# SuperScientificSoftwareLaboratory/TileSpMV

Measured on AMD Instinct MI355X. Metric: fp64 SpMV GFLOP/s (y = A*x, tiled format), higher is better.
Workload: dtype f64; 1 GPU; laplacian4096; rows=16777216, cols=16777216, nnz=83869696, partition=tile-row blocks, nnz-balanced, 1 rank(s), y_combine=none, tiles=5234176, x_panel_merge=0, x_slice_passes=0

## Files before the change

### tilespmv_amd/csrc/hip_plan.h

```cpp
#pragma once
#include <cstdint>

#include "host_util.h"

namespace tilespmv {

constexpr unsigned DESC_FMT_MASK = 7u;
constexpr unsigned DESC_FMT_NOP = 7u;
constexpr unsigned DESC_EOR = 8u;
constexpr int DESC_P1_SHIFT = 4;
constexpr int DESC_P2_SHIFT = 12;

#if defined(TILESPMV_F32)
struct ERec { unsigned v, w; };
#else
struct ERec { unsigned lo, hi, w; };
#endif
constexpr int ECHUNK = 64;
constexpr int SMALL_GRID_WORKGROUPS = 128;
constexpr int FB_DEST_BITS = 11;

struct Task {
    int tile_begin, tile_end;
    long long val_off;
    long long idx_off;
    int row;
    int partial;
};

struct FixRow { int row, first, count, pad; };

struct DevPlan {
    const uint2 *desc;
    const val_t *val;
    const unsigned char *idx;
    const Task *task;
    int ntasks;
    int rowA, colA;
    val_t *partial;
    const FixRow *fix;
    int nfix;
    const FixRow *fix_late;
    int nfix_late;
    const int4 *f_blk;
    const ERec *f_rec;
    const unsigned *f_base;
    int f_nblk;
    int f_ordered;
    int f_row0;
    int f_rows;
};

constexpr int FB_ROWS = 2048;
constexpr int FB_CAP = 6144;
constexpr int STRIP_MAX_ROWS = 8;
constexpr unsigned UNIT_EOR = 1u;
constexpr int UNIT_ROW_SHIFT = 1;
constexpr unsigned UNIT_ROWUNIT = 16u;
constexpr int UNIT_SHIFT_SHIFT = 29;
constexpr int ABSORB_SHIFT_MIN = -3, ABSORB_SHIFT_MAX = 3;
constexpr unsigned UNIT_DERIVED_CODE = 4u;
constexpr int UNIT_GROUP = 16 / (int)sizeof(val_t);
constexpr int UNIT_GROUP_NARROW = 4;
constexpr long long NT_STREAM_MIN_BYTES = 400ll << 20;
constexpr int DICT_MAX_BITS = 10;
constexpr int UNIT_FLAG_SHIFT = 24;

struct UDesc { unsigned w0, n0, n1; };

constexpr int POOL_KR_SHIFT = 28;
constexpr unsigned POOL_BASE_MASK = (1u << POOL_KR_SHIFT) - 1u;
constexpr int POOL_WORD_KR_SHIFT = 30;
__host__ __device__ inline int pool_word_base_bits(int npatterns)
{
    int ib = 1;
    while ((1 << ib) < npatterns) ib++;
    return POOL_WORD_KR_SHIFT - ib;
}
constexpr int POOL_MIN_FILL = sizeof(val_t) == 8 ? 12 : 10;
#ifndef TILESPMV_POOL_STRIP_ROWS
#define TILESPMV_POOL_STRIP_ROWS 4
#endif
constexpr int POOL_STRIP_ROWS = TILESPMV_POOL_STRIP_ROWS;
struct URow { unsigned r0, r1; };
constexpr unsigned POOL_WIDE_WINDOW = 256;
constexpr double POOL_WIDE_MAX_LINES = 3.5;

struct STask {
    int unit_begin, unit_end;
    int coo_begin, coo_end;
    int row;
    int partial;
    unsigned nounit_mask;
    int nrows;
};

struct DevStream {
    const UDesc *udesc;
    const URow *urow;
    const uint4 *ucol;
    const uint4 *pdict;
    int pooled;
    const val_t *uval;
    const val_t *cval;
    const int *ccol;
    const unsigned char *crow;
    const STask *task;
    int ntasks;
    int coo_heavy_min;
    int coo_ordered;
    int y_streaming;
    const int4 *wg_coo;
    const ERec *grec;
    const unsigned *gbase;
    int dest_bits;
    const uint4 *udict;
    int cb_bits;
    int nt_stream;
    int uval_narrow;
    const int *panel_off;
    int x_panels;
    int panel_merge;
    int n_groups;
    int slice_passes;
    int slice_ct;
    const UDesc *udesc_cb;
    const FixRow *ifix;
    unsigned *ifix_count;
};

struct DenseRow { int row, tile_begin, tile_end, partial; };
__host__ __device__ constexpr int dense_slot(int r, int c)
{
    return sizeof(val_t) == 8 ? ((c & 3) >> 1) * 128 + ((c >> 2) * 16 + r) * 2 + (c & 1) : ((c >> 2) * 16 + r) * 4 + (c & 3);
}

struct DevDense {
    const int *cb;
    const val_t *val;
    const DenseRow *rows;
    int nrows;
};

inline void tile_stream_sizes(int fmt, int p1, int p2, int *nv, int *ni)
{
    switch (fmt) {
    case TILESPMV_FMT_CSR: *nv = p1; *ni = 16 + (p1 + 1) / 2; break;
    case TILESPMV_FMT_COO: *nv = p1; *ni = p1; break;
    case TILESPMV_FMT_ELL: *nv = 16 * p1; *ni = 8 * p1; break;
    case TILESPMV_FMT_HYB: *nv = 16 * p1 + p2; *ni = 8 * p1 + p2; break;
    case TILESPMV_FMT_DNS: *nv = 256; *ni = 0; break;
    case TILESPMV_FMT_DNSROW: *nv = 16 * p1; *ni = p1; break;
    case TILESPMV_FMT_DNSCOL: *nv = 16 * p1; *ni = p1; break;
    default: *nv = 0; *ni = 0; break;
    }
}

hipError_t launch_units_half(const DevPlan &P, const DevStream &S, int entry_mode, int wg_strips, int lds_pad_bytes, int xcd_chunk, const val_t *x, val_t *y, hipStream_t st);

}
```

### tilespmv_amd/csrc/hip_units_kernel.h

```cpp
#pragma once
#include <hip/hip_runtime.h>

#include <type_traits>

#include "hip_plan.h"

namespace tilespmv {

typedef double lacc_t;

template <int CTRL>
__device__ __forceinline__ double dpp_mov(double v)
{
    int lo = __double2loint(v), hi = __double2hiint(v);
    lo = __builtin_amdgcn_update_dpp(0, lo, CTRL, 0xF, 0xF, false);
    hi = __builtin_amdgcn_update_dpp(0, hi, CTRL, 0xF, 0xF, false);
    return __hiloint2double(hi, lo);
}
template <int CTRL>
__device__ __forceinline__ float dpp_mov(float v)
{
    return __int_as_float(__builtin_amdgcn_update_dpp(0, __float_as_int(v), CTRL, 0xF, 0xF, false));
}
template <class T>
__device__ __forceinline__ T strip_allreduce(T v)
{
    v += dpp_mov<0x128>(v);
    v += dpp_mov<0x124>(v);
    v += dpp_mov<0x122>(v);
    v += dpp_mov<0x121>(v);
    return v;
}

__device__ __forceinline__ void wave_lds_fence()
{
    __builtin_amdgcn_fence(__ATOMIC_ACQ_REL, "wavefront");
    __builtin_amdgcn_wave_barrier();
}


template <bool NT, class T>
__device__ __forceinline__ T stream_load(const T *p)
{
    if constexpr (NT) return __builtin_nontemporal_load(p);
    else return *p;
}

__device__ __forceinline__ uint4 load_udesc(const UDesc *__restrict__ d, int i)
{
    const UDesc u = d[i];
    return make_uint4(u.w0, u.n0, u.w0, u.n1);
}

__device__ __forceinline__ uint4 load_udesc_raw(const UDesc *__restrict__ d, int i)
{
    const UDesc u = d[i];
    return make_uint4(u.w0, u.n0, u.n1, 0u);
}
__device__ __forceinline__ uint4 udesc_park_form(const uint4 raw) { return make_uint4(raw.x, raw.y, raw.x, raw.z); }

__device__ __forceinline__ uint4 udict_of(const DevStream &S, unsigned w) { return S.udict[(w << 5) >> (5 + S.cb_bits)]; }
__device__ __forceinline__ uint2 pool_desc(const DevStream &S, int i)
{
    const int b = S.cb_bits;
    if (b > 0) {
        const unsigned a = reinterpret_cast<const unsigned *>(S.udesc)[i];
        return make_uint2((a & ((1u << b) - 1u)) | ((a >> POOL_WORD_KR_SHIFT) << POOL_KR_SHIFT), (a << (32 - POOL_WORD_KR_SHIFT)) >> (32 - POOL_WORD_KR_SHIFT + b));
    }
    return reinterpret_cast<const uint2 *>(S.udesc)[i];
}
__device__ __forceinline__ uint4 udesc_expand(const DevStream &S, unsigned w, uint4 pat)
{
    const unsigned w0 = (w & ((1u << S.cb_bits) - 1u)) | ((w >> 27) << UNIT_FLAG_SHIFT) | pat.z;
    return make_uint4(w0, pat.x, w0, pat.y);
}
template <class X>
__device__ __forceinline__ X unit_x_use(X gathered, X prev, unsigned w0, int r)
{
    const X up = dpp_mov<0x12F>(prev);
    return ((w0 >> UNIT_SHIFT_SHIFT) == UNIT_DERIVED_CODE && r != 15) ? up : gathered;
}
__device__ __forceinline__ long long unit_x_base(unsigned w0) { return (long long)(w0 & 0xFFFFFFu) * 16 + ((int)w0 >> UNIT_SHIFT_SHIFT); }
__device__ __forceinline__ int unit_x_base32(unsigned w0) { return (int)((w0 & 0xFFFFFFu) << 4) + ((int)w0 >> UNIT_SHIFT_SHIFT); }
__device__ __forceinline__ unsigned x_index32(int base, unsigned off, int xlast) { return (unsigned)min(base + (int)off, xlast); }

constexpr int DCHUNK = 16;
typedef unsigned v4u_t __attribute__((ext_vector_type(4)));
typedef unsigned v2u_t __attribute__((ext_vector_type(2)));
#ifndef NT_Y
#define NT_Y 1
#endif
#ifndef WCOO_HEAVY_CT
#define WCOO_HEAVY_CT 6
#endif
#ifndef MV_MIN_WAVES
#define MV_MIN_WAVES 6
#endif
#ifndef ECOO2_MIN_WAVES
#define ECOO2_MIN_WAVES 6
#endif
#ifndef TILESPMV_UB
#define TILESPMV_UB 4
#endif
#ifndef UNITS_MIN_WAVES
#define UNITS_MIN_WAVES 8
#endif
#ifndef UNIT_X32
#define UNIT_X32 1
#endif
#ifndef UNIT_TAIL_HOT
#define UNIT_TAIL_HOT 1
#endif
#ifndef POOL_ECOO2_MIN_WAVES
#define POOL_ECOO2_MIN_WAVES 5
#endif
#ifndef POOL_MIN_WAVES
#define POOL_MIN_WAVES 7
#endif

__device__ __forceinline__ val_t erec_val(const ERec &r)
{
#if defined(TILESPMV_F32)
    return __uint_as_float(r.v);
#else
    return __hiloint2double((int)r.hi, (int)r.lo);
#endif
}

template <int CT>
__device__ __forceinline__ void wave_entry_trips(const DevStream &S, const val_t *__restrict__ x, lacc_t *swave, int lane, int gb, int ge, int chunk0, int cfirst)
{
    const int db = S.dest_bits;
    const unsigned dmask = (1u << db) - 1u;
    const int clast = chunk0 + ((ge - 1 - gb) >> 6);
    for (int e0 = gb + 64 * cfirst; e0 < ge; e0 += 64 * CT) {
        ERec rr[CT]; unsigned cb[CT]; val_t xx[CT];
#pragma unroll
        for (int q = 0; q < CT; q++) {
            rr[q] = S.grec[min(e0 + 64 * q + lane, ge - 1)];
            cb[q] = S.gbase[__builtin_amdgcn_readfirstlane(min(chunk0 + ((e0 - gb) >> 6) + q, clast))];
        }
#pragma unroll
        for (int q = 0; q < CT; q++) xx[q] = x[(size_t)(cb[q] + (rr[q].w >> db))];
#pragma unroll
        for (int q = 0; q < CT; q++)
            if (e0 + 64 * q + lane < ge) atomicAdd(&swave[rr[q].w & dmask], (lacc_t)(erec_val(rr[q]) * xx[q]));
    }
}

#ifndef WG_TRIP_PIPE
#define WG_TRIP_PIPE 0
#endif

template <int CT, int NT, bool NTL>
__device__ __forceinline__ void wg_entry_trips(const ERec *__restrict__ rec, const unsigned *__restrict__ base, int chunk0, int db, bool ordered,
                                               const val_t *__restrict__ x, lacc_t *sy, int tid, int gb, int ge, int gs = -1)
{
    if (gs < 0) gs = gb;
    const int e_first = gb + ((gs - gb) & ~63);
    const unsigned dmask = (1u << db) - 1u;
    const int wave = tid >> 6;
    const int clast = chunk0 + ((ge - 1 - gb) >> 6);
    ERec rr[CT]; unsigned cb[CT];
    auto load_trip = [&](int e0, ERec (&r)[CT], unsigned (&c)[CT]) {
#pragma unroll
        for (int q = 0; q < CT; q++) {
            if constexpr (NTL) {
                const unsigned *pw = reinterpret_cast<const unsigned *>(&rec[min(e0 + NT * q + tid, ge - 1)]);
                unsigned *rw = reinterpret_cast<unsigned *>(&r[q]);
#pragma unroll
                for (int z = 0; z < (int)(sizeof(ERec) / 4); z++) rw[z] = __builtin_nontemporal_load(pw + z);
            } else r[q] = rec[min(e0 + NT * q + tid, ge - 1)];
            c[q] = base[__builtin_amdgcn_readfirstlane(min(chunk0 + ((e0 - gb) >> 6) + (NT / 64) * q + wave, clast))];
        }
    };
    if (e_first < ge) load_trip(e_first, rr, cb);
    for (int e0 = e_first; e0 < ge; e0 += NT * CT) {
        val_t xx[CT];
        if (!WG_TRIP_PIPE && e0 > e_first) load_trip(e0, rr, cb);
#pragma unroll
        for (int q = 0; q < CT; q++) xx[q] = x[(size_t)(cb[q] + (rr[q].w >> db))];
        ERec rn[CT]; unsigned cn[CT];
        if (WG_TRIP_PIPE) load_trip(min(e0 + NT * CT, gb + (ge - 1 - gb) / (NT * CT) * (NT * CT)), rn, cn);
        if (ordered) {
            for (int w = 0; w < NT / 64; w++) {
                if (wave == w) {
#pragma unroll
                    for (int q = 0; q < CT; q++)
                        if (e0 + NT * q + tid < ge && e0 + NT * q + tid >= gs) atomicAdd(&sy[rr[q].w & dmask], (lacc_t)(erec_val(rr[q]) * xx[q]));
                }
                __syncthreads();
            }
        } else {
#pragma unroll
            for (int q = 0; q < CT; q++)
                if (e0 + NT * q + tid < ge && e0 + NT * q + tid >= gs) atomicAdd(&sy[rr[q].w & dmask], (lacc_t)(erec_val(rr[q]) * xx[q]));
        }
        if (WG_TRIP_PIPE) {
#pragma unroll
            for (int q = 0; q < CT; q++) { rr[q] = rn[q]; cb[q] = cn[q]; }
        }
    }
}

extern __shared__ __attribute__((aligned(16))) unsigned char s_dyn[];
#if defined(UNITS_KERNEL) != defined(UNITS_NARROW_FORM)
#error "hip_units_kernel.h: define UNITS_KERNEL and UNITS_NARROW_FORM together (or neither: k_units, floats)"
#endif
#ifndef UNITS_KERNEL
#define UNITS_KERNEL k_units
#define UNITS_NARROW_FORM 1
#endif
template <int UB, int ECOO, int GPB, bool CD, bool NTS, bool POOL = false, bool WIDE = false, bool NARROW = false>
__global__ __launch_bounds__(16 * GPB, ECOO == 1 ? 4 : ECOO == 2 ? (POOL ? POOL_ECOO2_MIN_WAVES : NARROW && UNITS_NARROW_FORM == 2 ? UNITS_MIN_WAVES : ECOO2_MIN_WAVES) : POOL ? (WIDE ? 6 : POOL_MIN_WAVES) : UNITS_MIN_WAVES) void UNITS_KERNEL(DevStream S, int rowA, int colA, int xcd_chunk, val_t *__restrict__ partial,
                                               const val_t *__restrict__ x, val_t *__restrict__ y)
{
    constexpr int VFORM = NARROW ? UNITS_NARROW_FORM : 0;
    static_assert(VFORM >= 0 && VFORM <= 2, "UNITS_NARROW_FORM: 1 or 2");
    static_assert(!NARROW || (sizeof(val_t) == 8 && !POOL && ECOO != 1 && GPB == 16 && NTS), "narrow values: fp64 classic plans, entry mode 0 / 2, 16 strips, nontemporal streams");
    constexpr int G = NARROW ? UNIT_GROUP_NARROW : UNIT_GROUP;
    static_assert(DCHUNK % UB == 0 && UB % G == 0, "a batch never straddles a descriptor chunk and is whole value groups");
    static_assert(GPB == 16 || (GPB == 32 && ECOO == 2) || (GPB == 8 && ECOO != 2 && !NTS), "512-thread workgroups exist for the workgroup entry mode only, 128-thread ones for small grids without it");
    static_assert(!(NTS && ECOO == 1), "nontemporal streams: large plans only (entry mode 1 = small grids)");
    static_assert(!POOL || GPB == 16 || GPB == 8, "pooled plans: 256-thread workgroups (128 on small grids)");
    static_assert(!WIDE || (POOL && !CD), "wide windows: pooled plans, 12-B descriptors + 16 B of column offsets");
    constexpr int GROUPS_PER_BLOCK = GPB;
    constexpr int SROWS = POOL ? POOL_STRIP_ROWS : STRIP_MAX_ROWS;
    constexpr bool NT = NTS;
#ifndef TILESPMV_NT_DESC
#define TILESPMV_NT_DESC 0
#endif
#ifndef TILESPMV_NT_COO0
#define TILESPMV_NT_COO0 0
#endif
    constexpr bool NT_DESC = NTS && TILESPMV_NT_DESC, NT_COO0 = NTS && TILESPMV_NT_COO0;
    constexpr bool PCOPY = POOL && sizeof(val_t) == 4;
    constexpr int SLAB = GROUPS_PER_BLOCK * SROWS * 16;
    __shared__ lacc_t s_yall[SLAB + (PCOPY ? SLAB + 16 : 0)];
    lacc_t (*s_y)[SROWS][16] = reinterpret_cast<lacc_t (*)[SROWS][16]>(&s_yall[0]);
    lacc_t *s_y1 = &s_yall[PCOPY ? SLAB + 16 : 0];
    __shared__ uint4 s_d[GROUPS_PER_BLOCK][DCHUNK];
    __shared__ uint2 s_r[POOL && !WIDE ? GROUPS_PER_BLOCK : 1][POOL && !WIDE ? DCHUNK : 1];
    __shared__ uint4 s_c[WIDE ? GROUPS_PER_BLOCK : 1][WIDE ? DCHUNK : 1];
    const int tid = threadIdx.x, r = tid & 15, g = tid >> 4;
    unsigned bid = blockIdx.x;
    if (xcd_chunk > 0) {
        const unsigned C = (unsigned)xcd_chunk, W = 8u * C, win = bid / W, off = bid % W, k = off & 7u;
        if ((win + 1) * W <= gridDim.x) bid = win * W + k * C + (off >> 3);
    }
    const long long task_id = (long long)bid * GROUPS_PER_BLOCK + g;
    const bool have = task_id < S.ntasks;
    constexpr bool WCOO = ECOO == 1;
    if (ECOO == 1) { if ((long long)bid * GROUPS_PER_BLOCK + (g & ~3) >= S.ntasks) return; }
    else if (ECOO == 0 && !have) return;
    int4 t0 = make_int4(0, 0, 0, 0), t1 = make_int4(0, -1, 0, 0);
    if (have) {
        t0 = reinterpret_cast<const int4 *>(S.task)[task_id * 2];
        t1 = reinterpret_cast<const int4 *>(S.task)[task_id * 2 + 1];
    }
    const int unit_begin = t0.x, unit_end = t0.y, coo_begin = t0.z, coo_end = t0.w;
    const int row0 = t1.x, part = t1.y, nrows = t1.w;
    const unsigned nounit = (unsigned)t1.z;
    const bool side = POOL || coo_end > coo_begin;
    if constexpr (POOL) {
        for (int k = 0; k < nrows; k++) { s_y[g][k][r] = 0; if constexpr (PCOPY) s_y1[(g * SROWS + k) * 16 + r] = 0; }
        wave_lds_fence();
    }
    typedef std::conditional_t<VFORM == 2, _Float16, std::conditional_t<VFORM == 1, float, val_t>> sval_t;
    typedef sval_t grp_t __attribute__((ext_vector_type(G)));
    const grp_t *__restrict__ ugrp = reinterpret_cast<const grp_t *>(S.uval) + r;
    const int last = unit_end - 1;
    const int last_grp = unit_begin + (unit_end - 1 - unit_begin) / G * G;
    const bool have_units = unit_begin < unit_end;
    const long long xlast = (long long)colA - 1;
    const int xlast32 = colA - 1;
    const int ncoo = coo_end - coo_begin;
    uint4 dcur = make_uint4(0u, 0u, 0u, 0u), dnext = dcur;
    uint2 rcur = make_uint2(0u, 0u), rnext = rcur;
    const uint2 *__restrict__ urw = reinterpret_cast<const uint2 *>(S.urow);
    uint4 ccur = make_uint4(0u, 0u, 0u, 0u), cnext = ccur;
    unsigned wnn = 0;
    const unsigned *__restrict__ udw = reinterpret_cast<const unsigned *>(S.udesc);
    uint2 wnn2 = make_uint2(0u, 0u);
    val_t v[UB];
    auto unit_prologue = [&]() {
        if (have_units) {
            if constexpr (CD && POOL) {
                const uint2 a = pool_desc(S, min(unit_begin + r, last)), b = pool_desc(S, min(unit_begin + DCHUNK + r, last));
                dcur.x = a.x; dcur.y = a.y; dnext.x = b.x; dnext.y = b.y;
            } else if constexpr (CD) {
                dcur.x = stream_load<NT_DESC>(udw + min(unit_begin + r, last));
                dnext.x = stream_load<NT_DESC>(udw + min(unit_begin + DCHUNK + r, last));
            } else {
                dcur = load_udesc_raw(S.udesc, min(unit_begin + r, last));
                dnext = load_udesc_raw(S.udesc, min(unit_begin + DCHUNK + r, last));
                if constexpr (WIDE) { ccur = S.ucol[min(unit_begin + r, last)]; cnext = S.ucol[min(unit_begin + DCHUNK + r, last)]; }
                else if constexpr (POOL) { rcur = urw[min(unit_begin + r, last)]; rnext = urw[min(unit_begin + DCHUNK + r, last)]; }
            }
#pragma unroll
            for (int k = 0; k < UB; k += G) {
                const grp_t pv = stream_load<NT>(ugrp + (long long)min(unit_begin + k, last_grp) * (16 / G));
#pragma unroll
                for (int q = 0; q < G; q++) v[k + q] = pv[q];
            }
        }
    };

    const uint2 *sd = reinterpret_cast<const uint2 *>(&s_d[g][0]) + (r >> 3);
    uint2 d[UB];
    unsigned rw[UB];
    val_t xv[UB];
    const unsigned *sr = reinterpret_cast<const unsigned *>(&s_r[POOL && !WIDE ? g : 0][0]) + (r >> 3);
    const unsigned char *sc = reinterpret_cast<const unsigned char *>(&s_c[WIDE ? g : 0][0]) + r;
    auto park_first = [&]() {
        if constexpr (CD && POOL) {
            const uint4 p0 = S.pdict[dcur.y], p1 = S.pdict[dnext.y];
            wnn2 = pool_desc(S, min(unit_begin + 2 * DCHUNK + r, last));
            s_d[g][r] = make_uint4(dcur.x, p0.x, dcur.x, p0.y); s_r[g][r] = make_uint2(p0.z, p0.w);
            dnext = make_uint4(dnext.x, p1.x, 0u, p1.y); rnext = make_uint2(p1.z, p1.w);
        } else if constexpr (CD) {
            const uint4 p0 = udict_of(S, dcur.x), p1 = udict_of(S, dnext.x);
            wnn = stream_load<NT_DESC>(udw + min(unit_begin + 2 * DCHUNK + r, last));
            dnext.y = p1.x; dnext.z = p1.z; dnext.w = p1.y;
            s_d[g][r] = udesc_expand(S, dcur.x, p0);
        } else s_d[g][r] = udesc_park_form(dcur);
        if constexpr (WIDE) s_c[g][r] = ccur;
        else if constexpr (POOL && !CD) s_r[g][r] = rcur;
    };
    auto fetch_batch = [&](int j0) {
#pragma unroll
        for (int k = 0; k < UB; k++) d[k] = sd[2 * (j0 + k)];
        if constexpr (WIDE) {
#pragma unroll
            for (int k = 0; k < UB; k++) rw[k] = d[k].y;
#pragma unroll
            for (int k = 0; k < UB; k++) {
                if constexpr (UNIT_X32) xv[k] = x[x_index32((int)(d[k].x & POOL_BASE_MASK), sc[16 * (j0 + k)], xlast32)];
                else xv[k] = x[min((long long)(d[k].x & POOL_BASE_MASK) + (long long)sc[16 * (j0 + k)], xlast)];
            }
            return;
        }
        if constexpr (POOL) {
#pragma unroll
            for (int k = 0; k < UB; k++) rw[k] = sr[2 * (j0 + k)];
#pragma unroll
            for (int k = 0; k < UB; k++) {
                if constexpr (UNIT_X32) xv[k] = x[x_index32((int)(d[k].x & POOL_BASE_MASK), (d[k].y >> (28 - 4 * (r & 7))) & 15u, xlast32)];
                else xv[k] = x[min((long long)(d[k].x & POOL_BASE_MASK) + (long long)((d[k].y >> (28 - 4 * (r & 7))) & 15u), xlast)];
            }
            return;
        }
#pragma unroll
        for (int k = 0; k < UB; k++) {
            const unsigned fl = d[k].x >> 24;
            const unsigned nib = (fl & UNIT_ROWUNIT) ? (unsigned)r : (d[k].y >> (28 - 4 * (r & 7))) & 15u;
            if ((d[k].x >> UNIT_SHIFT_SHIFT) == UNIT_DERIVED_CODE && r != 15) xv[k] = 0;
            else if constexpr (UNIT_X32) xv[k] = x[x_index32(unit_x_base32(d[k].x), nib, xlast32)];
            else xv[k] = x[min(unit_x_base(d[k].x) + nib, xlast)];
        }
    };

    if constexpr (ECOO == 2) {
        const int4 wr = S.wg_coo[bid];
        if (wr.y > wr.x) {
            if (side) for (int k = 0; k < nrows; k++) s_y[g][k][r] = 0;
            __syncthreads();
        } else if ((S.panel_merge > 0 || S.slice_passes > 0) && side) {
            for (int k = 0; k < nrows; k++) s_y[g][k][r] = 0;
            wave_lds_fence();
        }
        constexpr bool LATE_PROLOGUE = VFORM == 2;
        if constexpr (!LATE_PROLOGUE) unit_prologue();
        if (wr.y > wr.x) {
            int ge = wr.y;
            if (GPB == 16 && S.panel_merge > 0) ge = S.panel_off[(size_t)bid * (size_t)(S.x_panels + 1) + (size_t)min(S.x_panels, S.panel_merge)];
            if (GPB == 16 && S.slice_passes > 0) ge = wr.x;
            wg_entry_trips<WCOO_HEAVY_CT, 16 * GPB, NTS>(S.grec, S.gbase, wr.z, S.dest_bits, S.coo_ordered != 0, x, &s_y[0][0][0], tid, wr.x, ge);
            __syncthreads();
        }
        if constexpr (LATE_PROLOGUE) unit_prologue();
    } else if constexpr (WCOO) {
        constexpr int CT = 6;
        const int lane = tid & 63;
        const int4 wr = S.wg_coo[(long long)bid * (GROUPS_PER_BLOCK / 4) + (g >> 2)];
        const int tot = wr.y - wr.x;
        lacc_t *swave = &s_y[g & ~3][0][0];
        unit_prologue();
        ERec rr[CT]; unsigned cbase[CT]; val_t xx[CT];
        const int db = S.dest_bits;
        if (tot > 0) {
            if (side) for (int k = 0; k < nrows; k++) s_y[g][k][r] = 0;
            const int clast = wr.z + ((tot - 1) >> 6);
#pragma unroll
            for (int q = 0; q < CT; q++) {
                rr[q] = S.grec[min(wr.x + 64 * q + lane, wr.y - 1)];
                cbase[q] = S.gbase[__builtin_amdgcn_readfirstlane(min(wr.z + q, clast))];
            }
        }
        if (have_units) {
            park_first();
            wave_lds_fence();
            fetch_batch(0);
        } else if (tot > 0) wave_lds_fence();
        if (tot > 0) {
            const unsigned dmask = (1u << db) - 1u;
#pragma unroll
            for (int q = 0; q < CT; q++) xx[q] = x[(size_t)(cbase[q] + (rr[q].w >> db))];
#pragma unroll
            for (int q = 0; q < CT; q++)
                if (wr.x + 64 * q + lane < wr.y) atomicAdd(&swave[rr[q].w & dmask], (lacc_t)(erec_val(rr[q]) * xx[q]));
            if (tot > 64 * CT) wave_entry_trips<CT>(S, x, swave, lane, wr.x, wr.y, wr.z, CT);
            wave_lds_fence();
        }
    } else {
    constexpr int CT = 6;
    const bool coo_heavy = ncoo > S.coo_heavy_min;
    if (side) {
        for (int k = 0; k < nrows; k++) s_y[g][k][r] = 0;
        wave_lds_fence();
    }
    if (coo_heavy) {
        for (int e0 = coo_begin; e0 < coo_end; e0 += 16 * CT) {
            unsigned rb[CT]; int cc[CT]; val_t cv[CT], xx[CT];
#pragma unroll
            for (int q = 0; q < CT; q++) {
                const int e = min(e0 + 16 * q + r, coo_end - 1);
                rb[q] = S.crow[e]; cc[q] = S.ccol[e]; cv[q] = S.cval[e];
            }
#pragma unroll
            for (int q = 0; q < CT; q++) xx[q] = x[cc[q]];
#pragma unroll
            for (int q = 0; q < CT; q++)
                if (e0 + 16 * q + r < coo_end) atomicAdd(&s_y[g][rb[q] >> 4][rb[q] & 15u], (lacc_t)(cv[q] * xx[q]));
        }
        wave_lds_fence();
    }
    unsigned rb0 = 0; int cc0 = 0; val_t cv0 = 0;
    const bool coo0 = side && !coo_heavy && (coo_begin + r < coo_end);
    if (coo0) { rb0 = stream_load<NT_COO0>(S.crow + coo_begin + r); cc0 = stream_load<NT_COO0>(S.ccol + coo_begin + r); cv0 = stream_load<NT_COO0>(S.cval + coo_begin + r); }
    unit_prologue();
    if (side && !coo_heavy) {
        if (coo0) atomicAdd(&s_y[g][rb0 >> 4][rb0 & 15u], (lacc_t)(cv0 * x[cc0]));
        for (int e0 = coo_begin + 16; e0 < coo_end; e0 += 64) {
            unsigned rb[4]; int cc[4]; val_t cv[4], xx[4];
#pragma unroll
            for (int q = 0; q < 4; q++) {
                const int e = min(e0 + 16 * q + r, coo_end - 1);
                rb[q] = S.crow[e]; cc[q] = S.ccol[e]; cv[q] = S.cval[e];
            }
#pragma unroll
            for (int q = 0; q < 4; q++) xx[q] = x[cc[q]];
#pragma unroll
            for (int q = 0; q < 4; q++)
                if (e0 + 16 * q + r < coo_end) atomicAdd(&s_y[g][rb[q] >> 4][rb[q] & 15u], (lacc_t)(cv[q] * xx[q]));
        }
        wave_lds_fence();
    }
    }

    val_t acc = 0;
    auto retire = [&](val_t prod, unsigned flags, unsigned word1) {
        if constexpr (POOL) {
            const unsigned dest = ((flags >> (POOL_KR_SHIFT - 24)) & 7u) * 16u + ((word1 >> (28 - 4 * (r & 7))) & 15u);
            if constexpr (PCOPY) atomicAdd(((r & 1) ? s_y1 : &s_y[0][0][0]) + g * (SROWS * 16) + dest, (lacc_t)prod);
            else atomicAdd(&s_y[g][0][0] + dest, (lacc_t)prod);
            return;
        }
        if (flags & UNIT_ROWUNIT) {
            prod = strip_allreduce(prod);
            if (r != (int)(word1 & 15u)) prod = 0;
        }
        acc += prod;
        if (flags & UNIT_EOR) {
            const int kr = (int)((flags >> UNIT_ROW_SHIFT) & 7u);
            if constexpr (sizeof(val_t) == sizeof(lacc_t)) {
                lacc_t out = acc;
                if (side) out += s_y[g][kr][r];
                s_y[g][kr][r] = out;
            } else {
                val_t out = acc;
                if (side) out = (val_t)((lacc_t)acc + s_y[g][kr][r]);
                reinterpret_cast<val_t *>(&s_y[g][kr][0])[r] = out;
            }
            acc = 0;
        }
    };
    if (have_units) {
        if (ECOO != 1) {
            park_first();
            wave_lds_fence();
        }
        int chunk_end = unit_begin + DCHUNK;
        val_t xprev = 0;
        for (int u = unit_begin; u < unit_end; u += UB) {
            if (u == chunk_end) {
                wave_lds_fence();
                if constexpr (CD && POOL) { s_d[g][r] = make_uint4(dnext.x, dnext.y, dnext.x, dnext.w); s_r[g][r] = rnext; }
                else if constexpr (CD) s_d[g][r] = udesc_expand(S, dnext.x, make_uint4(dnext.y, dnext.w, dnext.z, 0u));
                else s_d[g][r] = udesc_park_form(dnext);
                if constexpr (WIDE) { s_c[g][r] = cnext; cnext = S.ucol[min(chunk_end + DCHUNK + r, last)]; }
                else if constexpr (POOL && !CD) { s_r[g][r] = rnext; rnext = urw[min(chunk_end + DCHUNK + r, last)]; }
                wave_lds_fence();
                chunk_end += DCHUNK;
                if constexpr (CD && POOL) {
                    const uint4 p = S.pdict[wnn2.y];
                    dnext = make_uint4(wnn2.x, p.x, 0u, p.y); rnext = make_uint2(p.z, p.w);
                    wnn2 = pool_desc(S, min(chunk_end + DCHUNK + r, last));
                } else if constexpr (CD) {
                    const uint4 p = udict_of(S, wnn);
                    dnext = make_uint4(wnn, p.x, p.z, p.y);
                    wnn = stream_load<NT_DESC>(udw + min(chunk_end + DCHUNK + r, last));
                } else dnext = load_udesc_raw(S.udesc, min(chunk_end + r, last));
            }
            if (!(ECOO == 1 && u == unit_begin)) fetch_batch(u - (chunk_end - DCHUNK));
            sval_t vn[UB];
#pragma unroll
            for (int k = 0; k < UB; k += G) {
                const grp_t *pa = ugrp + (long long)min(u + UB + k, last_grp) * (16 / G);
                if constexpr (UNIT_TAIL_HOT) pa = (u + UB + k <= last_grp) ? pa : reinterpret_cast<const grp_t *>(S.uval);
                const grp_t pv = stream_load<NT>(pa);
#pragma unroll
                for (int q = 0; q < G; q++) vn[k + q] = pv[q];
            }
#pragma unroll
            for (int k = 0; k < UB; k++)
            {
                if constexpr (POOL) {
                    retire((u + k < unit_end) ? v[k] * xv[k] : (val_t)0, d[k].x >> 24, rw[k]);
                } else {
                    const val_t xu = unit_x_use(xv[k], xprev, d[k].x, r);
                    xprev = xu;
                    if (u + k < unit_end) retire(v[k] * xu, d[k].x >> 24, d[k].y);
                }
            }
#pragma unroll
            for (int k = 0; k < UB; k++) v[k] = vn[k];
        }
    }
    if constexpr (POOL) {
        wave_lds_fence();
        if constexpr (PCOPY) {
            for (int k = 0; k < nrows; k++) s_y[g][k][r] += s_y1[(g * SROWS + k) * 16 + r];
            wave_lds_fence();
        }
    }
    if (part >= 0) {
        val_t out = acc;
        if (side) out = (val_t)((lacc_t)acc + s_y[g][0][r]);
        if (S.ifix_count == nullptr || nounit == 0xFFFFFFFFu) {
            partial[(long long)part * 16 + r] = out;
        } else {
            __hip_atomic_store(&partial[(long long)part * 16 + r], out, __ATOMIC_RELAXED, __HIP_MEMORY_SCOPE_AGENT);
            __builtin_amdgcn_fence(__ATOMIC_RELEASE, "wavefront");
            asm volatile("s_waitcnt vmcnt(0)" ::: "memory");
            const FixRow f = S.ifix[nounit];
            unsigned prev = 0;
            if (r == 0) prev = __hip_atomic_fetch_add(&S.ifix_count[nounit], 1u, __ATOMIC_RELAXED, __HIP_MEMORY_SCOPE_AGENT);
            prev = (unsigned)__shfl((int)prev, tid & 48, 64);
            __builtin_amdgcn_fence(__ATOMIC_ACQUIRE, "wavefront");
            if (prev == (unsigned)f.count - 1u) {
                val_t sum = 0;
                for (int k0 = 0; k0 < f.count; k0 += 8) {
                    val_t sv[8];
#pragma unroll
                    for (int j = 0; j < 8; j++)
                        sv[j] = __hip_atomic_load(&partial[(long long)(f.first + min(k0 + j, f.count - 1)) * 16 + r], __ATOMIC_RELAXED, __HIP_MEMORY_SCOPE_AGENT);
#pragma unroll
                    for (int j = 0; j < 8; j++) if (k0 + j < f.count) sum += sv[j];
                }
                const long long yi = (long long)f.row * 16 + r;
                if (yi < rowA) y[yi] = sum;
                if (r == 0) __hip_atomic_store(&S.ifix_count[nounit], 0u, __ATOMIC_RELAXED, __HIP_MEMORY_SCOPE_AGENT);
            }
        }
    } else {
        if constexpr (POOL) {
            if constexpr (sizeof(val_t) != sizeof(lacc_t)) {
                for (int k = 0; k < nrows; k++) {
                    const val_t o = (val_t)s_y[g][k][r];
                    reinterpret_cast<val_t *>(&s_y[g][k][0])[r] = o;
                }
            }
        } else if constexpr (sizeof(val_t) == sizeof(lacc_t)) {
            if (!side) {
                unsigned m = nounit;
                while (m) { const int kr = __ffs((int)m) - 1; m &= m - 1; s_y[g][kr][r] = 0; }
            }
        } else {
            unsigned m = nounit;
            while (m) {
                const int kr = __ffs((int)m) - 1; m &= m - 1;
                const val_t o = side ? (val_t)s_y[g][kr][r] : (val_t)0;
                reinterpret_cast<val_t *>(&s_y[g][kr][0])[r] = o;
            }
        }
        wave_lds_fence();
        constexpr int VEC = 16 / (int)sizeof(val_t);
        const lacc_t *res = &s_y[g][0][0];
        const long long ybase = (long long)row0 * 16;
        for (int i = r * VEC; i < 16 * nrows; i += 16 * VEC) {
            if constexpr (sizeof(val_t) == sizeof(lacc_t)) {
                if (ybase + i + VEC <= rowA) {
                    if (NT_Y && S.y_streaming) __builtin_nontemporal_store(*reinterpret_cast<const v4u_t *>(res + i), reinterpret_cast<v4u_t *>(y + ybase + i));
                    else *reinterpret_cast<uint4 *>(y + ybase + i) = *reinterpret_cast<const uint4 *>(res + i);
                } else {
#pragma unroll
                    for (int q = 0; q < VEC; q++) if (ybase + i + q < rowA) y[ybase + i + q] = (val_t)res[i + q];
                }
            } else {
                const val_t *rf = reinterpret_cast<const val_t *>(res) + (i >> 4) * 32 + (i & 15);
                if (ybase + i + VEC <= rowA) {
                    if (NT_Y && S.y_streaming) __builtin_nontemporal_store(*reinterpret_cast<const v4u_t *>(rf), reinterpret_cast<v4u_t *>(y + ybase + i));
                    else *reinterpret_cast<uint4 *>(y + ybase + i) = *reinterpret_cast<const uint4 *>(rf);
                } else {
#pragma unroll
                    for (int q = 0; q < VEC; q++) if (ybase + i + q < rowA) y[ybase + i + q] = rf[q];
                }
            }
        }
    }
}

}
```

Before: 1610 GFLOP/s.

## Repack parked unit descriptors and restructure classic unit loop with scalar row-unit path

Non-pooled units now park a compact descriptor word that folds the x base, end-of-row, row-unit and derived flags together, so the x byte offset comes from a shift, an alignbit and a min. The classic loop is split from the pooled one and walks chunks by pointer, without the per-iteration chunk test. Row-unit handling is gated by a wave-uniform scalar flag, derived-x values use DPP moves, and row indices come from a precomputed list of remaining rows. Together these aim to cut VALU and address math in the hot loop, at the cost of more intricate code and tighter bit-width limits on x indices.

```diff
diff --git a/tilespmv_amd/csrc/hip_plan.h b/tilespmv_amd/csrc/hip_plan.h
--- a/tilespmv_amd/csrc/hip_plan.h
+++ b/tilespmv_amd/csrc/hip_plan.h
@@ -65,6 +65,10 @@
 constexpr long long NT_STREAM_MIN_BYTES = 400ll << 20;
 constexpr int DICT_MAX_BITS = 10;
 constexpr int UNIT_FLAG_SHIFT = 24;
+constexpr int UPARK_BASE_SHIFT = 2, UPARK_BASE_BITS = 29;
+constexpr unsigned UPARK_EOR = 1u;
+constexpr unsigned UPARK_ROWUNIT = 2u;
+constexpr unsigned UPARK_DERIVED = 1u << 31;
 
 struct UDesc { unsigned w0, n0, n1; };
 
diff --git a/tilespmv_amd/csrc/hip_units_kernel.h b/tilespmv_amd/csrc/hip_units_kernel.h
--- a/tilespmv_amd/csrc/hip_units_kernel.h
+++ b/tilespmv_amd/csrc/hip_units_kernel.h
@@ -32,6 +32,29 @@
     return v;
 }
 
+template <int CTRL>
+__device__ __forceinline__ double dpp_rotate(double v)
+{
+    int lo = __double2loint(v), hi = __double2hiint(v);
+    lo = __builtin_amdgcn_mov_dpp(lo, CTRL, 0xF, 0xF, false);
+    hi = __builtin_amdgcn_mov_dpp(hi, CTRL, 0xF, 0xF, false);
+    return __hiloint2double(hi, lo);
+}
+template <int CTRL>
+__device__ __forceinline__ float dpp_rotate(float v)
+{
+    return __int_as_float(__builtin_amdgcn_mov_dpp(__float_as_int(v), CTRL, 0xF, 0xF, false));
+}
+template <class T>
+__device__ __forceinline__ T strip_allreduce_rotating(T v)
+{
+    v += dpp_rotate<0x128>(v);
+    v += dpp_rotate<0x124>(v);
+    v += dpp_rotate<0x122>(v);
+    v += dpp_rotate<0x121>(v);
+    return v;
+}
+
 __device__ __forceinline__ void wave_lds_fence()
 {
     __builtin_amdgcn_fence(__ATOMIC_ACQ_REL, "wavefront");
@@ -60,6 +83,12 @@
 __device__ __forceinline__ uint4 udesc_park_form(const uint4 raw) { return make_uint4(raw.x, raw.y, raw.x, raw.z); }
 
 __device__ __forceinline__ uint4 udict_of(const DevStream &S, unsigned w) { return S.udict[(w << 5) >> (5 + S.cb_bits)]; }
+struct UDict3 { unsigned x, y, z; };
+__device__ __forceinline__ uint4 udict3_of(const DevStream &S, unsigned w)
+{
+    const UDict3 p = *reinterpret_cast<const UDict3 *>(&S.udict[(w << 5) >> (5 + S.cb_bits)]);
+    return make_uint4(p.x, p.y, p.z, 0u);
+}
 __device__ __forceinline__ uint2 pool_desc(const DevStream &S, int i)
 {
     const int b = S.cb_bits;
@@ -83,6 +112,47 @@
 __device__ __forceinline__ long long unit_x_base(unsigned w0) { return (long long)(w0 & 0xFFFFFFu) * 16 + ((int)w0 >> UNIT_SHIFT_SHIFT); }
 __device__ __forceinline__ int unit_x_base32(unsigned w0) { return (int)((w0 & 0xFFFFFFu) << 4) + ((int)w0 >> UNIT_SHIFT_SHIFT); }
 __device__ __forceinline__ unsigned x_index32(int base, unsigned off, int xlast) { return (unsigned)min(base + (int)off, xlast); }
+
+__device__ __forceinline__ uint4 upark_form(unsigned w0, unsigned n0, unsigned n1, bool null_unit)
+{
+    const unsigned fl = w0 >> UNIT_FLAG_SHIFT;
+    unsigned a = ((unsigned)unit_x_base32(w0) << (32 - UPARK_BASE_BITS)) >> (32 - UPARK_BASE_BITS - UPARK_BASE_SHIFT);
+    if (!null_unit) a |= (fl & UNIT_EOR) | ((fl & UNIT_ROWUNIT) ? UPARK_ROWUNIT : 0u) | ((w0 >> UNIT_SHIFT_SHIFT) == UNIT_DERIVED_CODE ? UPARK_DERIVED : 0u);
+    return make_uint4(a, n0, a, n1);
+}
+__device__ __forceinline__ unsigned upark_nib_rot(int r) { return (unsigned)(28 - 4 * (r & 7) - 3) & 31u; }
+__device__ __forceinline__ unsigned upark_nib8(unsigned nibbles, unsigned nib_rot) { return __builtin_amdgcn_alignbit(nibbles, nibbles, nib_rot) & (15u << 3); }
+template <class V>
+__device__ __forceinline__ unsigned upark_x_offset(unsigned a, unsigned nib8, unsigned xlast8)
+{
+    static_assert(UPARK_BASE_SHIFT == 2 && UPARK_BASE_BITS == 29, "word A << 1 = base * 8 + flags");
+    static_assert(UPARK_ROWUNIT == 2u, "the loop extracts the row-unit flag as bit 1 of word A");
+    const unsigned o = min((a << 1) + nib8, xlast8);
+    return sizeof(V) == 8 ? (o & ~7u) : ((o >> 1) & ~3u);
+}
+__device__ __forceinline__ bool scalar_flag(int uniform)
+{
+    int s = __builtin_amdgcn_readfirstlane(uniform);
+    asm volatile("" : "+s"(s));
+    return s != 0;
+}
+template <class V>
+__device__ __forceinline__ V unwritten_register()
+{
+    V t;
+    asm volatile("" : "=v"(t));
+    return t;
+}
+__device__ __forceinline__ double derived_x(double gathered, double prev)
+{
+    const int lo = __builtin_amdgcn_update_dpp(__double2loint(gathered), __double2loint(prev), 0x101, 0xF, 0xF, false);
+    const int hi = __builtin_amdgcn_update_dpp(__double2hiint(gathered), __double2hiint(prev), 0x101, 0xF, 0xF, false);
+    return __hiloint2double(hi, lo);
+}
+__device__ __forceinline__ float derived_x(float gathered, float prev)
+{
+    return __int_as_float(__builtin_amdgcn_update_dpp(__float_as_int(gathered), __float_as_int(prev), 0x101, 0xF, 0xF, false));
+}
 
 constexpr int DCHUNK = 16;
 typedef unsigned v4u_t __attribute__((ext_vector_type(4)));
@@ -274,6 +344,14 @@
     const bool have_units = unit_begin < unit_end;
     const long long xlast = (long long)colA - 1;
     const int xlast32 = colA - 1;
+    const unsigned xlast8 = (unsigned)min(xlast32, (1 << 28) + 18) * 8u + 7u;
+    const unsigned nib_rot = POOL ? 0u : upark_nib_rot(r);
+    bool park_rowunits = false;
+    auto park_classic = [&](unsigned w0, unsigned n0, unsigned n1, int first_unit) {
+        const bool null_unit = first_unit + r > last;
+        park_rowunits = __builtin_amdgcn_ballot_w64(!null_unit && ((w0 >> UNIT_FLAG_SHIFT) & UNIT_ROWUNIT)) != 0;
+        s_d[g][r] = upark_form(w0, n0, n1, null_unit);
+    };
     const int ncoo = coo_end - coo_begin;
     uint4 dcur = make_uint4(0u, 0u, 0u, 0u), dnext = dcur;
     uint2 rcur = make_uint2(0u, 0u), rnext = rcur;
@@ -283,6 +361,7 @@
     const unsigned *__restrict__ udw = reinterpret_cast<const unsigned *>(S.udesc);
     uint2 wnn2 = make_uint2(0u, 0u);
     val_t v[UB];
+    grp_t vg[UB / G];
     auto unit_prologue = [&]() {
         if (have_units) {
             if constexpr (CD && POOL) {
@@ -300,6 +379,7 @@
 #pragma unroll
             for (int k = 0; k < UB; k += G) {
                 const grp_t pv = stream_load<NT>(ugrp + (long long)min(unit_begin + k, last_grp) * (16 / G));
+                vg[k / G] = pv;
 #pragma unroll
                 for (int q = 0; q < G; q++) v[k + q] = pv[q];
             }
@@ -319,15 +399,17 @@
             s_d[g][r] = make_uint4(dcur.x, p0.x, dcur.x, p0.y); s_r[g][r] = make_uint2(p0.z, p0.w);
             dnext = make_uint4(dnext.x, p1.x, 0u, p1.y); rnext = make_uint2(p1.z, p1.w);
         } else if constexpr (CD) {
-            const uint4 p0 = udict_of(S, dcur.x), p1 = udict_of(S, dnext.x);
+            const uint4 p0 = udict3_of(S, dcur.x), p1 = udict3_of(S, dnext.x);
             wnn = stream_load<NT_DESC>(udw + min(unit_begin + 2 * DCHUNK + r, last));
             dnext.y = p1.x; dnext.z = p1.z; dnext.w = p1.y;
-            s_d[g][r] = udesc_expand(S, dcur.x, p0);
-        } else s_d[g][r] = udesc_park_form(dcur);
+            const uint4 e = udesc_expand(S, dcur.x, p0);
+            park_classic(e.x, e.y, e.w, unit_begin);
+        } else if constexpr (POOL) s_d[g][r] = udesc_park_form(dcur);
+        else park_classic(dcur.x, dcur.y, dcur.z, unit_begin);
         if constexpr (WIDE) s_c[g][r] = ccur;
         else if constexpr (POOL && !CD) s_r[g][r] = rcur;
     };
-    auto fetch_batch = [&](int j0) {
+    auto fetch_pooled = [&](int j0) {
 #pragma unroll
         for (int k = 0; k < UB; k++) d[k] = sd[2 * (j0 + k)];
         if constexpr (WIDE) {
@@ -340,23 +422,30 @@
             }
             return;
         }
-        if constexpr (POOL) {
-#pragma unroll
-            for (int k = 0; k < UB; k++) rw[k] = sr[2 * (j0 + k)];
-#pragma unroll
-            for (int k = 0; k < UB; k++) {
-                if constexpr (UNIT_X32) xv[k] = x[x_index32((int)(d[k].x & POOL_BASE_MASK), (d[k].y >> (28 - 4 * (r & 7))) & 15u, xlast32)];
-                else xv[k] = x[min((long long)(d[k].x & POOL_BASE_MASK) + (long long)((d[k].y >> (28 - 4 * (r & 7))) & 15u), xlast)];
-            }
-            return;
-        }
+#pragma unroll
+        for (int k = 0; k < UB; k++) rw[k] = sr[2 * (j0 + k)];
 #pragma unroll
         for (int k = 0; k < UB; k++) {
-            const unsigned fl = d[k].x >> 24;
-            const unsigned nib = (fl & UNIT_ROWUNIT) ? (unsigned)r : (d[k].y >> (28 - 4 * (r & 7))) & 15u;
-            if ((d[k].x >> UNIT_SHIFT_SHIFT) == UNIT_DERIVED_CODE && r != 15) xv[k] = 0;
-            else if constexpr (UNIT_X32) xv[k] = x[x_index32(unit_x_base32(d[k].x), nib, xlast32)];
-            else xv[k] = x[min(unit_x_base(d[k].x) + nib, xlast)];
+            if constexpr (UNIT_X32) xv[k] = x[x_index32((int)(d[k].x & POOL_BASE_MASK), (d[k].y >> (28 - 4 * (r & 7))) & 15u, xlast32)];
+            else xv[k] = x[min((long long)(d[k].x & POOL_BASE_MASK) + (long long)((d[k].y >> (28 - 4 * (r & 7))) & 15u), xlast)];
+        }
+    };
+    auto fetch_batch = [&](const uint2 *sdu, int rowunits, val_t xprev) {
+#pragma unroll
+        for (int k = 0; k < UB; k++) d[k] = sdu[2 * k];
+        if (scalar_flag(rowunits)) {
+            unsigned ident = (unsigned)r & 8u;
+            asm volatile("" : "+v"(ident));
+            ident = 0x01234567u + ident * 0x11111111u;
+#pragma unroll
+            for (int k = 0; k < UB; k++) if (__builtin_amdgcn_ubfe(d[k].x, 1, 1)) d[k].y = ident;
+        }
+#pragma unroll
+        for (int k = 0; k < UB; k++) {
+            const unsigned nib = upark_nib8(d[k].y, nib_rot);
+            xv[k] = unwritten_register<val_t>();
+            if (k == 0) xv[k] = derived_x(xv[k], xprev);
+            if ((int)d[k].x >= 0 || r == 15) xv[k] = *reinterpret_cast<const val_t *>(reinterpret_cast<const char *>(x) + upark_x_offset<val_t>(d[k].x, nib, xlast8));
         }
     };
 
@@ -400,7 +489,8 @@
         if (have_units) {
             park_first();
             wave_lds_fence();
-            fetch_batch(0);
+            if constexpr (POOL) fetch_pooled(0);
+            else fetch_batch(sd, __builtin_amdgcn_readfirstlane((int)park_rowunits), (val_t)0);
         } else if (tot > 0) wave_lds_fence();
         if (tot > 0) {
             const unsigned dmask = (1u << db) - 1u;
@@ -458,29 +548,36 @@
     }
     }
 
+    unsigned rows_left = 076543210u;
+    if (!POOL && part < 0 && ((unsigned)t1.z & ((1u << STRIP_MAX_ROWS) - 1u)) != 0) {
+        rows_left = 0;
+        for (int k = STRIP_MAX_ROWS - 1; k >= 0; k--) if (!(((unsigned)t1.z >> k) & 1u)) rows_left = (rows_left << 3) | (unsigned)k;
+    }
     val_t acc = 0;
-    auto retire = [&](val_t prod, unsigned flags, unsigned word1) {
-        if constexpr (POOL) {
-            const unsigned dest = ((flags >> (POOL_KR_SHIFT - 24)) & 7u) * 16u + ((word1 >> (28 - 4 * (r & 7))) & 15u);
-            if constexpr (PCOPY) atomicAdd(((r & 1) ? s_y1 : &s_y[0][0][0]) + g * (SROWS * 16) + dest, (lacc_t)prod);
-            else atomicAdd(&s_y[g][0][0] + dest, (lacc_t)prod);
-            return;
-        }
-        if (flags & UNIT_ROWUNIT) {
-            prod = strip_allreduce(prod);
-            if (r != (int)(word1 & 15u)) prod = 0;
-        }
+    const unsigned row0_nrows = (unsigned)row0 | ((unsigned)nrows << 28);
+    auto retire_pooled = [&](val_t prod, unsigned flags, unsigned word1) {
+        const unsigned dest = ((flags >> (POOL_KR_SHIFT - 24)) & 7u) * 16u + ((word1 >> (28 - 4 * (r & 7))) & 15u);
+        if constexpr (PCOPY) atomicAdd(((r & 1) ? s_y1 : &s_y[0][0][0]) + g * (SROWS * 16) + dest, (lacc_t)prod);
+        else atomicAdd(&s_y[g][0][0] + dest, (lacc_t)prod);
+    };
+    auto retire = [&](val_t prod, unsigned flags) {
+#pragma clang fp contract(off)
         acc += prod;
-        if (flags & UNIT_EOR) {
-            const int kr = (int)((flags >> UNIT_ROW_SHIFT) & 7u);
+        if (flags & UPARK_EOR) {
+            const int kr = (int)(rows_left & 7u);
+            rows_left >>= 3;
+            unsigned t = (unsigned)tid;
+            if constexpr (!NARROW && sizeof(val_t) == 8) asm volatile("" : "+v"(t));
+            lacc_t *const row = &s_y[0][0][0] + ((t >> 4) * SROWS + (unsigned)kr) * 16u;
+            const unsigned rr = t & 15u;
             if constexpr (sizeof(val_t) == sizeof(lacc_t)) {
                 lacc_t out = acc;
-                if (side) out += s_y[g][kr][r];
-                s_y[g][kr][r] = out;
+                if (side) out += row[rr];
+                row[rr] = out;
             } else {
                 val_t out = acc;
-                if (side) out = (val_t)((lacc_t)acc + s_y[g][kr][r]);
-                reinterpret_cast<val_t *>(&s_y[g][kr][0])[r] = out;
+                if (side) out = (val_t)((lacc_t)acc + row[rr]);
+                reinterpret_cast<val_t *>(row)[rr] = out;
             }
             acc = 0;
         }
@@ -490,51 +587,95 @@
             park_first();
             wave_lds_fence();
         }
-        int chunk_end = unit_begin + DCHUNK;
-        val_t xprev = 0;
-        for (int u = unit_begin; u < unit_end; u += UB) {
-            if (u == chunk_end) {
+        if constexpr (POOL) {
+            int chunk_end = unit_begin + DCHUNK;
+            for (int u = unit_begin; u < unit_end; u += UB) {
+                if (u == chunk_end) {
+                    wave_lds_fence();
+                    if constexpr (CD) { s_d[g][r] = make_uint4(dnext.x, dnext.y, dnext.x, dnext.w); s_r[g][r] = rnext; }
+                    else s_d[g][r] = udesc_park_form(dnext);
+                    if constexpr (WIDE) { s_c[g][r] = cnext; cnext = S.ucol[min(chunk_end + DCHUNK + r, last)]; }
+                    else if constexpr (!CD) { s_r[g][r] = rnext; rnext = urw[min(chunk_end + DCHUNK + r, last)]; }
+                    wave_lds_fence();
+                    chunk_end += DCHUNK;
+                    if constexpr (CD) {
+                        const uint4 p = S.pdict[wnn2.y];
+                        dnext = make_uint4(wnn2.x, p.x, 0u, p.y); rnext = make_uint2(p.z, p.w);
+                        wnn2 = pool_desc(S, min(chunk_end + DCHUNK + r, last));
+                    } else dnext = load_udesc_raw(S.udesc, min(chunk_end + r, last));
+                }
+                if (!(ECOO == 1 && u == unit_begin)) fetch_pooled(u - (chunk_end - DCHUNK));
+                sval_t vn[UB];
+#pragma unroll
+                for (int k = 0; k < UB; k += G) {
+                    const grp_t *pa = ugrp + (long long)min(u + UB + k, last_grp) * (16 / G);
+                    if constexpr (UNIT_TAIL_HOT) pa = (u + UB + k <= last_grp) ? pa : reinterpret_cast<const grp_t *>(S.uval);
+                    const grp_t pv = stream_load<NT>(pa);
+#pragma unroll
+                    for (int q = 0; q < G; q++) vn[k + q] = pv[q];
+                }
+#pragma unroll
+                for (int k = 0; k < UB; k++) retire_pooled((u + k < unit_end) ? v[k] * xv[k] : (val_t)0, d[k].x >> 24, rw[k]);
+#pragma unroll
+                for (int k = 0; k < UB; k++) v[k] = vn[k];
+            }
+        } else {
+            val_t xprev = 0;
+            const grp_t *vnext = ugrp + ((long long)unit_begin + UB) * (16 / G);
+            int rowunits = __builtin_amdgcn_readfirstlane((int)park_rowunits);
+            int u = unit_begin;
+            const uint2 *sdu = sd;
+            for (;;) {
+#pragma clang loop unroll(disable)
+                for (int b = 0; b < DCHUNK / UB && u <= last; b++, u += UB) {
+#pragma clang fp contract(off)
+                    if (!(ECOO == 1 && u == unit_begin)) fetch_batch(sdu, rowunits, xprev);
+                    grp_t vgn[UB / G];
+#pragma unroll
+                    for (int k = 0; k < UB; k += G) {
+                        const grp_t *pa;
+                        if constexpr (UNIT_TAIL_HOT) pa = (u + UB + k <= last) ? vnext + k * (16 / G) : reinterpret_cast<const grp_t *>(S.uval);
+                        else pa = ugrp + (long long)min(u + UB + k, last_grp) * (16 / G);
+                        vgn[k / G] = stream_load<NT>(pa);
+                    }
+                    vnext += UB * (16 / G);
+                    val_t prod[UB];
+#pragma unroll
+                    for (int k = 0; k < UB; k++) {
+                        if constexpr (VFORM == 2 || sizeof(val_t) == 4) {
+                            if (k > 0) { const val_t up = derived_x(xv[k], xv[k - 1]); xv[k] = (int)d[k].x < 0 ? up : xv[k]; }
+                        } else if (k > 0 && (int)d[k].x < 0) xv[k] = derived_x(xv[k], xv[k - 1]);
+                        prod[k] = (val_t)vg[k / G][k % G] * xv[k];
+                    }
+                    if (scalar_flag(rowunits)) {
+#pragma unroll
+                        for (int k = 0; k < UB; k++)
+                            if (__builtin_amdgcn_ubfe(d[k].x, 1, 1)) {
+                                prod[k] = strip_allreduce_rotating(prod[k]);
+                                if (r != (int)(sdu[2 * k].y & 15u)) prod[k] = 0;
+                            }
+                    }
+#pragma unroll
+                    for (int k = 0; k < UB; k++)
+                        if (k < G || u + k <= last) retire(prod[k], d[k].x);
+#pragma unroll
+                    for (int k = 0; k < UB / G; k++) vg[k] = vgn[k];
+                    xprev = xv[UB - 1];
+                    sdu += 2 * UB;
+                }
+                if (u > last) break;
+                sdu -= 2 * DCHUNK;
                 wave_lds_fence();
-                if constexpr (CD && POOL) { s_d[g][r] = make_uint4(dnext.x, dnext.y, dnext.x, dnext.w); s_r[g][r] = rnext; }
-                else if constexpr (CD) s_d[g][r] = udesc_expand(S, dnext.x, make_uint4(dnext.y, dnext.w, dnext.z, 0u));
-                else s_d[g][r] = udesc_park_form(dnext);
-                if constexpr (WIDE) { s_c[g][r] = cnext; cnext = S.ucol[min(chunk_end + DCHUNK + r, last)]; }
-                else if constexpr (POOL && !CD) { s_r[g][r] = rnext; rnext = urw[min(chunk_end + DCHUNK + r, last)]; }
+                if constexpr (CD) { const uint4 e = udesc_expand(S, dnext.x, make_uint4(dnext.y, dnext.w, dnext.z, 0u)); park_classic(e.x, e.y, e.w, u); }
+                else park_classic(dnext.x, dnext.y, dnext.z, u);
                 wave_lds_fence();
-                chunk_end += DCHUNK;
-                if constexpr (CD && POOL) {
-                    const uint4 p = S.pdict[wnn2.y];
-                    dnext = make_uint4(wnn2.x, p.x, 0u, p.y); rnext = make_uint2(p.z, p.w);
-                    wnn2 = pool_desc(S, min(chunk_end + DCHUNK + r, last));
-                } else if constexpr (CD) {
-                    const uint4 p = udict_of(S, wnn);
+                if constexpr (CD) {
+                    const uint4 p = udict3_of(S, wnn);
                     dnext = make_uint4(wnn, p.x, p.z, p.y);
-                    wnn = stream_load<NT_DESC>(udw + min(chunk_end + DCHUNK + r, last));
-                } else dnext = load_udesc_raw(S.udesc, min(chunk_end + r, last));
-            }
-            if (!(ECOO == 1 && u == unit_begin)) fetch_batch(u - (chunk_end - DCHUNK));
-            sval_t vn[UB];
-#pragma unroll
-            for (int k = 0; k < UB; k += G) {
-                const grp_t *pa = ugrp + (long long)min(u + UB + k, last_grp) * (16 / G);
-                if constexpr (UNIT_TAIL_HOT) pa = (u + UB + k <= last_grp) ? pa : reinterpret_cast<const grp_t *>(S.uval);
-                const grp_t pv = stream_load<NT>(pa);
-#pragma unroll
-                for (int q = 0; q < G; q++) vn[k + q] = pv[q];
-            }
-#pragma unroll
-            for (int k = 0; k < UB; k++)
-            {
-                if constexpr (POOL) {
-                    retire((u + k < unit_end) ? v[k] * xv[k] : (val_t)0, d[k].x >> 24, rw[k]);
-                } else {
-                    const val_t xu = unit_x_use(xv[k], xprev, d[k].x, r);
-                    xprev = xu;
-                    if (u + k < unit_end) retire(v[k] * xu, d[k].x >> 24, d[k].y);
-                }
-            }
-#pragma unroll
-            for (int k = 0; k < UB; k++) v[k] = vn[k];
+                    wnn = stream_load<NT_DESC>(udw + min(u + 2 * DCHUNK + r, last));
+                } else dnext = load_udesc_raw(S.udesc, min(u + DCHUNK + r, last));
+                rowunits = __builtin_amdgcn_readfirstlane((int)park_rowunits);
+            }
         }
     }
     if constexpr (POOL) {
@@ -597,8 +738,9 @@
         wave_lds_fence();
         constexpr int VEC = 16 / (int)sizeof(val_t);
         const lacc_t *res = &s_y[g][0][0];
-        const long long ybase = (long long)row0 * 16;
-        for (int i = r * VEC; i < 16 * nrows; i += 16 * VEC) {
+        const long long ybase = (long long)(POOL ? row0 : (int)(row0_nrows & 0x0FFFFFFFu)) * 16;
+        const int nrows_y = POOL ? nrows : (int)(row0_nrows >> 28);
+        for (int i = r * VEC; i < 16 * nrows_y; i += 16 * VEC) {
             if constexpr (sizeof(val_t) == sizeof(lacc_t)) {
                 if (ybase + i + VEC <= rowA) {
                     if (NT_Y && S.y_streaming) __builtin_nontemporal_store(*reinterpret_cast<const v4u_t *>(res + i), reinterpret_cast<v4u_t *>(y + ybase + i));
```

Result: no change. 1636 GFLOP/s, median of 6 (+1.6%).
